# kuldeepbrd1/graspLDM

Measured on AMD Instinct MI355X. Metric: grasps/sec whole-node (1024-pt cloud, 100 DDIM steps), higher is better.
Workload: dtype f32 (GEMMs as split-f16 x3 partial products on the f16 matrix pipe, f32 accumulation; GroupNorm / LayerNorm / attention / scheduler in f32); 1 GPU; LDM mode, 256 synthetic 1024-pt clouds per GPU x 20 grasps, 100 DDIM steps: BASELINE.json configs[2] per GPU (configs[3] = this per-GPU workload on 8 GPUs); experiment=fpc, clouds_per_gpu=256, grasps_per_cloud=20, points=1024, ddim_steps=100, encoder=PVCNNEncoder (shipped fpc config), parallelism=cloud-sharded x1, weights=synthetic recipe seed 0, streams=3

## Files before the change

### graspldm_amd/csrc/quad_narrow.h

```cpp
#ifndef GLDM_QUAD_NARROW_H_
#define GLDM_QUAD_NARROW_H_

#ifdef GLDM_DEBUG_KNOBS
__device__ long long g_q_stamp[4][16];
#define GLDM_QSTAMP(c, i) do { if (blockIdx.x == 0 && (c).lane == 0) g_q_stamp[(c).wave & 3][i] = (long long)__builtin_readcyclecounter(); } while (0)
#else
#define GLDM_QSTAMP(c, i) do {} while (0)
#endif

template <int CTRL>
__device__ __forceinline__ float dpp_zero(float x) {
  return __int_as_float(__builtin_amdgcn_update_dpp(0, __float_as_int(x), CTRL, 0xf, 0xf, true));
}
template <int CTRL>
__device__ __forceinline__ u32x4 dpp_zero4(const u32x4 &v) {
  u32x4 o;
#pragma unroll
  for (int i = 0; i < 4; ++i) o[i] = (unsigned)__builtin_amdgcn_update_dpp(0, (int)v[i], CTRL, 0xf, 0xf, true);
  return o;
}
__device__ __forceinline__ float pos_sum(float v) {
  v += dpp_mov<0x124>(v);
  return v + dpp_mov<0x128>(v);
}
__device__ __forceinline__ float pos_max(float v) { return dpp_max<0x128>(dpp_max<0x124>(v)); }
#define GLDM_DPP8_STAGE1(op, i, j) "v_" op "_f32_dpp %" #i ", %" #j ", %" #j " row_ror:4 row_mask:0xf bank_mask:0xf\n\t"
#define GLDM_DPP8_STAGE2(op, i) "v_" op "_f32_dpp %" #i ", %" #i ", %" #i " row_ror:8 row_mask:0xf bank_mask:0xf\n\t"
#define GLDM_DPP8(op)                                                                                                  \
  "s_nop 1\n\t"                                                                                                         \
  GLDM_DPP8_STAGE1(op, 0, 8) GLDM_DPP8_STAGE1(op, 1, 9) GLDM_DPP8_STAGE1(op, 2, 10) GLDM_DPP8_STAGE1(op, 3, 11)          \
  GLDM_DPP8_STAGE1(op, 4, 12) GLDM_DPP8_STAGE1(op, 5, 13) GLDM_DPP8_STAGE1(op, 6, 14) GLDM_DPP8_STAGE1(op, 7, 15)        \
  GLDM_DPP8_STAGE2(op, 0) GLDM_DPP8_STAGE2(op, 1) GLDM_DPP8_STAGE2(op, 2) GLDM_DPP8_STAGE2(op, 3)                        \
  GLDM_DPP8_STAGE2(op, 4) GLDM_DPP8_STAGE2(op, 5) GLDM_DPP8_STAGE2(op, 6) GLDM_DPP8_STAGE2(op, 7)
#define GLDM_DPP8_OPERANDS                                                                                             \
  : "=&v"(r[0]), "=&v"(r[1]), "=&v"(r[2]), "=&v"(r[3]), "=&v"(r[4]), "=&v"(r[5]), "=&v"(r[6]), "=&v"(r[7])            \
  : "v"(x[0]), "v"(x[1]), "v"(x[2]), "v"(x[3]), "v"(x[4]), "v"(x[5]), "v"(x[6]), "v"(x[7])
#define GLDM_DPP8_STAGE1I(op, i) "v_" op "_f32_dpp %" #i ", %" #i ", %" #i " row_ror:4 row_mask:0xf bank_mask:0xf\n\t"
__device__ __forceinline__ void pos_max8(float (&x)[8]) {
  asm("s_nop 1\n\t"
      GLDM_DPP8_STAGE1I("max", 0) GLDM_DPP8_STAGE1I("max", 1) GLDM_DPP8_STAGE1I("max", 2) GLDM_DPP8_STAGE1I("max", 3)
      GLDM_DPP8_STAGE1I("max", 4) GLDM_DPP8_STAGE1I("max", 5) GLDM_DPP8_STAGE1I("max", 6) GLDM_DPP8_STAGE1I("max", 7)
      GLDM_DPP8_STAGE2("max", 0) GLDM_DPP8_STAGE2("max", 1) GLDM_DPP8_STAGE2("max", 2) GLDM_DPP8_STAGE2("max", 3)
      GLDM_DPP8_STAGE2("max", 4) GLDM_DPP8_STAGE2("max", 5) GLDM_DPP8_STAGE2("max", 6) GLDM_DPP8_STAGE2("max", 7)
      : "+v"(x[0]), "+v"(x[1]), "+v"(x[2]), "+v"(x[3]), "+v"(x[4]), "+v"(x[5]), "+v"(x[6]), "+v"(x[7]));
}
__device__ __forceinline__ void pos_sum8(const float (&x)[8], float (&r)[8]) {
  asm(GLDM_DPP8("add") GLDM_DPP8_OPERANDS);
}
__device__ __forceinline__ float kq_sum(float v) { return half_sum(row_pair_sum(v)); }
__device__ __forceinline__ float kq_max(float v) { return half_max(row_pair_max(v)); }

__device__ __forceinline__ void qsplit8(const f32x4 &a, const f32x4 &b, u32x4 (&pl)[kSplit]) {
  unsigned h, l;
  split_f16x2(a[0], a[1], h, l); pl[0][0] = h; pl[1][0] = l;
  split_f16x2(a[2], a[3], h, l); pl[0][1] = h; pl[1][1] = l;
  split_f16x2(b[0], b[1], h, l); pl[0][2] = h; pl[1][2] = l;
  split_f16x2(b[2], b[3], h, l); pl[0][3] = h; pl[1][3] = l;
}

enum { QM_OUT0 = 0, QM_SS2, QM_C1_2, QM_C2_2, QM_SS3, QM_C1_3, QM_C2_3, QM_QKV1, QM_OUT1, QM_DOWN1,
       QM_SS4, QM_C1_4, QM_C2_4, QM_SS5, QM_C1_5, QM_C2_5, QM_QKV2, QM_OUT2, QM_DOWN2, QM_COUNT };
struct QOff { int mat, a, b; };
constexpr QOff qconv_frag(int mat, int MT, int KB, int i, int mt0 = 0) {
  const int st = i / MT, mi = i % MT, kb = st / 3, t = st % 3;
  const int f = (mt0 + mi) * 3 * KB + t * KB + kb;
  return QOff{mat, 2048 * f, 2048 * f + 1024};
}
constexpr QOff qrb_frag(int mss, int MT, int KB, int i) {
  if (i < MT) return QOff{mss, 1024 * i, 1024 * (MT + i)};
  i -= MT;
  if (i < 3 * KB * MT) return qconv_frag(mss + 1, MT, KB, i);
  return qconv_frag(mss + 2, MT, KB, i - 3 * KB * MT);
}
constexpr int qrb_len(int MT, int KB) { return MT + 6 * KB * MT; }
constexpr QOff qatt_frag(int mqkv, int MT, int KB, int i) {
  const int per = 6 * KB + MT, h = i / per, r = i % per;
  if (r < 6 * KB) {
    const int mt6 = r / KB, kb = r % KB, part = mt6 / 2, half = mt6 % 2;
    const int f = (2 * h + half + 8 * part) * KB + kb;
    return QOff{mqkv, 2048 * f, 2048 * f + 1024};
  }
  const int f = (r - 6 * KB) * 4 + h;
  return QOff{mqkv + 1, 2048 * f, 2048 * f + 1024};
}
constexpr int qatt_len(int MT, int KB) { return 4 * (6 * KB + MT); }
constexpr int qlevel_len(int MT, int KB) { return 2 * qrb_len(MT, KB) + qatt_len(MT, KB) + 2 * MT * 3 * KB; }
constexpr QOff qlevel_frag(int m0, int MT, int KB, int DP, int i) {
  if (i < qrb_len(MT, KB)) return qrb_frag(m0, MT, KB, i);
  i -= qrb_len(MT, KB);
  if (i < qrb_len(MT, KB)) return qrb_frag(m0 + 3, MT, KB, i);
  i -= qrb_len(MT, KB);
  if (i < qatt_len(MT, KB)) return qatt_frag(m0 + 6, MT, KB, i);
  i -= qatt_len(MT, KB);
  const int pass = i / (DP * 3 * KB);
  return qconv_frag(m0 + 8, DP, KB, i % (DP * 3 * KB), DP * pass);
}
constexpr int kQN0 = 0;
constexpr int kQN1 = 4;
constexpr int kQN2 = kQN1 + qlevel_len(2, 1);
constexpr int kQNEnd = kQN2 + qlevel_len(4, 2);
constexpr QOff qstream_off(int n) {
  if (n < kQN1) return QOff{QM_OUT0, 2048 * n, 2048 * n + 1024};
  if (n < kQN2) return qlevel_frag(QM_SS2, 2, 1, 4, n - kQN1);
  return qlevel_frag(QM_SS4, 4, 2, 4, n - kQN2);
}

constexpr int kQG = 4;
constexpr int kQS = 32;
constexpr int kQGroups = kQNEnd / kQG;
static_assert(kQNEnd % kQG == 0 && kQS % kQG == 0, "whole groups");
constexpr int kQR = 6;
constexpr int kQSpinMax = 1 << 20;
__host__ __device__ constexpr int qslot_floats(int s) { return (s < 16 ? PG<4>::kH : PG<4>::kX + 4 * PG<4>::kBlockFloats) + (s & 15) * 512; }
static_assert(PG<4>::kH + 16 * 512 <= PG<4>::kX && PG<4>::kX + 4 * PG<4>::kBlockFloats + 16 * 512 <= 512 * 64, "slot regions");
typedef __attribute__((address_space(3))) int lds_i;
struct QStream4 {
  static constexpr int kEnd = kQNEnd, kGroups = kQGroups;
  static constexpr QOff off(int n) { return qstream_off(n); }
  __host__ __device__ static constexpr int slot_floats(int s) { return qslot_floats(s); }
};

struct QRing {
  u32x4 s[kQR][2];
  float *lds;
  lds_i *sync;
  int lane, quad;
  int flag;
  int spins = 0;
};
__device__ __forceinline__ int lds_poll(const lds_i *p) {
  int v;
  asm volatile("ds_read_b32 %0, %1\n\ts_waitcnt lgkmcnt(0)" : "=v"(v) : "v"(p) : "memory");
  return __builtin_amdgcn_readfirstlane(v);
}
template <int N, class ST = QStream4>
__device__ __forceinline__ void qring_load(QRing &ring) {
  if constexpr (N < ST::kEnd) {
    if constexpr (N % kQG == 0) {
      constexpr int g = N / kQG;
#if defined(GLDM_DEBUG_KNOBS) && defined(GLDM_QEXP_DUP)
      if (false) {
#else
      if (__builtin_expect(ring.flag != g + 1, 0)) {
#endif
        for (int spin = 0; spin < kQSpinMax && lds_poll(ring.sync + (g & 7)) != g + 1; ++spin) {
          __builtin_amdgcn_s_sleep(1);
#ifdef GLDM_DEBUG_KNOBS
          ++ring.spins;
#endif
        }
      }
      if constexpr (g + 1 < ST::kGroups) ring.flag = *(volatile lds_i *)(ring.sync + ((g + 1) & 7));
    }
#if defined(GLDM_DEBUG_KNOBS) && defined(GLDM_QEXP_NOLOAD)
    if (N >= kQR) return;
#endif
    const lds_u4 *slot = (const lds_u4 *)(ring.lds + ST::slot_floats(N % kQS)) + ring.lane;
    ring.s[N % kQR][0] = slot[0];
    ring.s[N % kQR][1] = slot[64];
  }
}
template <int N, class ST = QStream4>
__device__ __forceinline__ f32x4 qring_mfma(QRing &ring, const u32x4 (&b)[kSplit], f32x4 acc) {
#if defined(GLDM_DEBUG_KNOBS) && defined(GLDM_QEXP_NOMFMA)
  acc[0] += __uint_as_float(ring.s[N % kQR][0][0] ^ b[0][0]);
#else
  acc = mfma_split(ring.s[N % kQR], b, acc);
#endif
  if constexpr (N % kQG == kQG - 1) ring.sync[16 + 64 * ring.quad + ring.lane] = N / kQG + 1;
  if constexpr (N >= 1) qring_load<N - 1 + kQR, ST>(ring);
  return acc;
}

typedef __attribute__((address_space(3))) void lds_void;
typedef __attribute__((address_space(1))) const void glob_void;
__device__ __forceinline__ void quad_build_table(const gldm_r1d_desc &d, int *qtab, int tid, int nthreads) {
  const int mbf[QM_COUNT] = {d.lv[0].out_wq,
                             d.rb[2].ss_w, d.rb[2].c1_wq, d.rb[2].c2_wq, d.rb[3].ss_w, d.rb[3].c1_wq, d.rb[3].c2_wq,
                             d.lv[1].qkvn_wq, d.lv[1].out_wq, d.lv[1].down_wq,
                             d.rb[4].ss_w, d.rb[4].c1_wq, d.rb[4].c2_wq, d.rb[5].ss_w, d.rb[5].c1_wq, d.rb[5].c2_wq,
                             d.lv[2].qkvn_wq, d.lv[2].out_wq, d.lv[2].down_wq};
  for (int n = tid; n < kQNEnd; n += nthreads) {
    const QOff o = qstream_off(n);
    int base = 0;
#pragma unroll
    for (int m = 0; m < QM_COUNT; ++m) base = o.mat == m ? mbf[m] * 4 : base;
    qtab[2 * n] = base + o.a;
    qtab[2 * n + 1] = base + o.b;
  }
}
template <class ST = QStream4>
__device__ __forceinline__ void quad_loader(const Ctx &c) {
  using GG = Geo<64>;
  lds_i *sync = (lds_i *)(c.lds + GG::kMiscQ);
  const lds_i *qtab = (const lds_i *)(c.lds + GG::kMiscQTab);
  const char *wb = reinterpret_cast<const char *>(c.w) + c.lane * 16;
  for (int g = c.wave - 4; g < ST::kGroups; g += 4) {
    if (g >= 8) {
      for (int spin = 0; spin < kQSpinMax; ++spin) {
        const int d0 = lds_poll(sync + 16), d1 = lds_poll(sync + 80), d2 = lds_poll(sync + 144), d3 = lds_poll(sync + 208);
        if (min(min(d0, d1), min(d2, d3)) >= g - 7) break;
        __builtin_amdgcn_s_sleep(2);
      }
    }
    const int s0 = (g & 7) * kQG;
#pragma unroll
    for (int f = 0; f < kQG; ++f) {
      const int n = g * kQG + f;
      const int oa = __builtin_amdgcn_readfirstlane(qtab[2 * n]), ob = __builtin_amdgcn_readfirstlane(qtab[2 * n + 1]);
      const int sl = s0 + f;
      float *slot = c.lds + ST::slot_floats(sl);
      __builtin_amdgcn_global_load_lds((glob_void *)(wb + oa), (lds_void *)slot, 16, 0, 0);
      __builtin_amdgcn_global_load_lds((glob_void *)(wb + ob), (lds_void *)(slot + 256), 16, 0, 0);
    }
    asm volatile("s_waitcnt vmcnt(0)" ::: "memory");
    if (c.lane == 0) sync[g & 7] = g + 1;
  }
}

template <int N0, int MT, int KB, int SH = 4, class ST = QStream4>
__device__ __forceinline__ void qconv3(QRing &ring, const u32x4 (&xp)[KB][kSplit], f32x4 (&acc)[MT]) {
  using std::integral_constant;
  auto body = [&](auto st_c) {
    constexpr int st = decltype(st_c)::value, kb = st / 3, t = st % 3;
    u32x4 bs[kSplit];
#pragma unroll
    for (int pl = 0; pl < kSplit; ++pl)
      bs[pl] = t == 1 ? xp[kb][pl] : (t == 0 ? dpp_zero4<0x110 + SH>(xp[kb][pl]) : dpp_zero4<0x100 + SH>(xp[kb][pl]));
    auto per_m = [&](auto mi_c) {
      constexpr int mi = decltype(mi_c)::value;
      acc[mi] = qring_mfma<N0 + st * MT + mi, ST>(ring, bs, acc[mi]);
    };
    per_m(integral_constant<int, 0>{});
    if constexpr (MT > 1) per_m(integral_constant<int, 1>{});
    if constexpr (MT > 2) { per_m(integral_constant<int, 2>{}); per_m(integral_constant<int, 3>{}); }
    __builtin_amdgcn_sched_barrier(0);
  };
  body(integral_constant<int, 0>{}); body(integral_constant<int, 1>{}); body(integral_constant<int, 2>{});
  if constexpr (KB > 1) { body(integral_constant<int, 3>{}); body(integral_constant<int, 4>{}); body(integral_constant<int, 5>{}); }
}

template <int MT, int CPG>
__device__ __forceinline__ void qgn_stats(const f32x4 (&acc)[MT], float (&mean)[MT], float (&var)[MT]) {
  static_assert(CPG == 8 || CPG == 16, "groups of half an m-tile or a whole one");
  constexpr float inv_n = 1.0f / (float)(CPG * 4);
#pragma unroll
  for (int mi = 0; mi < MT; ++mi) {
    float s = (acc[mi][0] + acc[mi][1]) + (acc[mi][2] + acc[mi][3]);
    s = row_pair_sum(pos_sum(s));
    if (CPG == 16) s = half_sum(s);
    const float m = s * inv_n;
    float v = 0.f;
#pragma unroll
    for (int r = 0; r < 4; ++r) {
      const float d = acc[mi][r] - m;
      v = fmaf(d, d, v);
    }
    v = row_pair_sum(pos_sum(v));
    if (CPG == 16) v = half_sum(v);
    mean[mi] = m;
    var[mi] = v * inv_n;
  }
}

struct QRb { int c1_b, n1_w, n1_b, c2_b, n2_w, n2_b, ss_b; };

template <int N0, int MT, int KB>
__device__ __forceinline__ void quad_resblock(const Ctx &c, QRing &ring, const QRb &rb, f32x4 (&xr)[MT],
                                              u32x4 (&xp)[KB][kSplit], int smp) {
  using GG = Geo<64>;
  using std::integral_constant;
  constexpr int C = 16 * MT, CPG = C / 4;
  const int kq = c.lane >> 4;
  const float *w = c.w;
  const lds_f *Gs = (const lds_f *)(c.lds + GG::kMiscG) + smp * 16;
  float gb[4];
#pragma unroll
  for (int j = 0; j < 4; ++j) gb[j] = Gs[4 * j + kq];
  f32x4 sc[MT], sh[MT], g1[MT], be1[MT], b1[MT];
#pragma unroll
  for (int mi = 0; mi < MT; ++mi) {
    const int row0 = 16 * mi + 4 * kq;
    sc[mi] = *reinterpret_cast<const f32x4 *>(w + rb.ss_b + row0);
    sh[mi] = *reinterpret_cast<const f32x4 *>(w + rb.ss_b + C + row0);
    b1[mi] = *reinterpret_cast<const f32x4 *>(w + rb.c1_b + row0);
    g1[mi] = *reinterpret_cast<const f32x4 *>(w + rb.n1_w + row0);
    be1[mi] = *reinterpret_cast<const f32x4 *>(w + rb.n1_b + row0);
  }
  {
    auto ss_m = [&](auto mi_c) {
      constexpr int mi = decltype(mi_c)::value;
      const u32x4 a_sc = ring.s[(N0 + mi) % kQR][0], a_sh = ring.s[(N0 + mi) % kQR][1];
#pragma unroll
      for (int j = 0; j < 4; ++j) {
        sc[mi] = __builtin_amdgcn_mfma_f32_16x16x4f32(__uint_as_float(a_sc[j]), gb[j], sc[mi], 0, 0, 0);
        sh[mi] = __builtin_amdgcn_mfma_f32_16x16x4f32(__uint_as_float(a_sh[j]), gb[j], sh[mi], 0, 0, 0);
      }
      if constexpr (N0 + mi >= 1) qring_load<N0 + mi - 1 + kQR>(ring);
    };
    ss_m(integral_constant<int, 0>{}); ss_m(integral_constant<int, 1>{});
    if constexpr (MT > 2) { ss_m(integral_constant<int, 2>{}); ss_m(integral_constant<int, 3>{}); }
  }
// ... 218 lines not shown
  const int i = lane & 15, kq = lane >> 4;
  f32x4 f = *reinterpret_cast<const f32x4 *>(w + off + ((kq * 16 + (i >> 2)) * 4));
  if (i & 3) f = f32x4{0.f, 0.f, 0.f, 0.f};
  return f;
}
__device__ __forceinline__ float q4_conv(const f32x4 &wt, float bias, float x) {
  f32x4 acc = f32x4{bias, 0.f, 0.f, 0.f};
  acc = __builtin_amdgcn_mfma_f32_16x16x4f32(wt[0], dpp_zero<0x114>(x), acc, 0, 0, 0);
  acc = __builtin_amdgcn_mfma_f32_16x16x4f32(wt[1], x, acc, 0, 0, 0);
  acc = __builtin_amdgcn_mfma_f32_16x16x4f32(wt[2], dpp_zero<0x104>(x), acc, 0, 0, 0);
  return acc[0];
}
__device__ __forceinline__ float q4_gn(float y, float gamma, float beta) {
  const float m = pos_sum(y) * 0.25f;
  const float d = y - m;
  const float rs = __builtin_amdgcn_rsqf(pos_sum(d * d) * 0.25f + 1e-5f);
  return d * rs * gamma + beta;
}
struct QRb4W { f32x4 w1, w2, wss; float b1, g1, be1, b2, g2, be2, ssb0, ssb1; };
__device__ __forceinline__ QRb4W quad_resblock4_load(const Ctx &c, const QRb4 &rb) {
  const int i = c.lane & 15, kq = c.lane >> 4;
  const float *w = c.w;
  QRb4W p;
  p.w1 = q4_weights(w, rb.c1_w, c.lane);
  p.w2 = q4_weights(w, rb.c2_w, c.lane);
  const int srow = (i & 3) == 0 ? (i >> 2) : 4 + (i >> 2);
  p.wss = *reinterpret_cast<const f32x4 *>(w + rb.ss_w + ((kq * 16 + srow) * 4));
  if ((i & 3) > 1) p.wss = f32x4{0.f, 0.f, 0.f, 0.f};
  p.b1 = w[rb.c1_b + kq]; p.g1 = w[rb.n1_w + kq]; p.be1 = w[rb.n1_b + kq];
  p.b2 = w[rb.c2_b + kq]; p.g2 = w[rb.n2_w + kq]; p.be2 = w[rb.n2_b + kq];
  p.ssb0 = w[rb.ss_b + kq]; p.ssb1 = w[rb.ss_b + 4 + kq];
  return p;
}
__device__ __forceinline__ float quad_resblock4(const Ctx &c, const QRb4W &p, float x, int smp) {
  using GG = Geo<64>;
  const int kq = c.lane >> 4;
  f32x4 ss = f32x4{p.ssb0, p.ssb1, 0.f, 0.f};
  const lds_f *Gs = (const lds_f *)(c.lds + GG::kMiscG) + smp * 16;
#pragma unroll
  for (int j = 0; j < 4; ++j) ss = __builtin_amdgcn_mfma_f32_16x16x4f32(p.wss[j], Gs[4 * j + kq], ss, 0, 0, 0);
  float y = q4_conv(p.w1, p.b1, x);
  y = silu(q4_gn(y, p.g1, p.be1) * ss[0] + ss[1]);
  float z = q4_conv(p.w2, p.b2, y);
  z = silu(q4_gn(z, p.g2, p.be2));
  return x + z;
}

struct QLv4 { int qkvn_w, out_b, ln2_g; };

__device__ __forceinline__ float quad_attention4(const Ctx &c, QRing &ring, const QLv4 &lv, float x) {
  using std::integral_constant;
  const int kq = c.lane >> 4;
  const float *w = c.w;
  float fq[kHeads][6];
#pragma unroll
  for (int h = 0; h < kHeads; ++h)
#pragma unroll
    for (int t = 0; t < 6; ++t)
      fq[h][t] = w[lv.qkvn_w + ((2 * h + (t & 1) + 8 * (t >> 1)) * 64 + c.lane) * 4] * (t < 4 ? 1.44269504088896340736f : 1.0f);
  const float outb = w[lv.out_b + kq], g2 = w[lv.ln2_g + kq];
  const float mean = kq_sum(x) * 0.25f;
  const float d = x - mean;
  const float xn = d * __builtin_amdgcn_rsqf(kq_sum(d * d) * 0.25f + 1e-5f);
  f32x4 oacc = f32x4{outb, 0.f, 0.f, 0.f};
  auto head = [&](auto h_c) {
    constexpr int h = decltype(h_c)::value;
    f32x4 qkv[6];
#pragma unroll
    for (int t = 0; t < 6; ++t) qkv[t] = __builtin_amdgcn_mfma_f32_16x16x4f32(fq[h][t], xn, f32x4{0.f, 0.f, 0.f, 0.f}, 0, 0, 0);
    f32x4 o[2];
    const f32x4 qa[2] = {qkv[0], qkv[1]}, ka[2] = {qkv[2], qkv[3]}, va[2] = {qkv[4], qkv[5]};
    quad_attention_head<true>(qa, ka, va, o);
    u32x4 op[kSplit];
    qsplit8(o[0], o[1], op);
    oacc = qring_mfma<kQN0 + h>(ring, op, oacc);
  };
  head(integral_constant<int, 0>{}); head(integral_constant<int, 1>{}); head(integral_constant<int, 2>{}); head(integral_constant<int, 3>{});
  const float y = oacc[0];
  const float m2 = kq_sum(y) * 0.25f;
  const float d2 = y - m2;
  return x + d2 * __builtin_amdgcn_rsqf(kq_sum(d2 * d2) * 0.25f + 1e-5f) * g2;
}

typedef __attribute__((address_space(4))) const gldm_r1d_desc kernarg_desc;
#define GLDM_QDESC() asm volatile("" : "+s"(dk))
__device__ __forceinline__ void quad_narrow_levels(const Ctx &c, kernarg_desc *dk) {
  using GG = Geo<64>;
  using std::integral_constant;
  const int q = c.wave & 3, col = c.lane & 15, kq = c.lane >> 4;
  const int p = col >> 2, sl = col & 3;
  const int smp = 4 * q + sl;
  const int pmcol = 16 * p + smp;
  const float *w = c.w;
  QRing ring;
  ring.lds = c.lds;
  ring.sync = (lds_i *)(c.lds + GG::kMiscQ);
  ring.lane = c.lane;
  ring.quad = q;
  ring.flag = 0;
  GLDM_QSTAMP(c, 0);
  qring_load<0>(ring); qring_load<1>(ring); qring_load<2>(ring); qring_load<3>(ring); qring_load<4>(ring); qring_load<5>(ring);
  static_assert(kQR == 6, "priming loads");
#define GLDM_QRB4(i) QRb4{dk->rb[i].c1_w, dk->rb[i].c1_b, dk->rb[i].n1_w, dk->rb[i].n1_b, dk->rb[i].c2_w, dk->rb[i].c2_b, dk->rb[i].n2_w, dk->rb[i].n2_b, dk->rb[i].ss_w, dk->rb[i].ss_b}
#define GLDM_QRB(i) QRb{dk->rb[i].c1_b, dk->rb[i].n1_w, dk->rb[i].n1_b, dk->rb[i].c2_b, dk->rb[i].n2_w, dk->rb[i].n2_b, dk->rb[i].ss_b}
#define GLDM_QLV(i) QLv{dk->lv[i].qkvn_s, dk->lv[i].out_b, dk->lv[i].ln2_g}
  GLDM_QDESC();
  const QRb4W p0 = quad_resblock4_load(c, GLDM_QRB4(0)), p1 = quad_resblock4_load(c, GLDM_QRB4(1));
  float x = ((const lds_f *)(c.lds + GG::kBufX))[pswz(kq, pmcol)];
  x = quad_resblock4(c, p0, x, smp);
  GLDM_QSTAMP(c, 1);
  x = quad_resblock4(c, p1, x, smp);
  GLDM_QSTAMP(c, 2);
  GLDM_QDESC();
  x = quad_attention4(c, ring, QLv4{dk->lv[0].qkvn_w, dk->lv[0].out_b, dk->lv[0].ln2_g}, x);
  GLDM_QSTAMP(c, 3);
  f32x4 x32[2];
  u32x4 xp32[1][kSplit];
  {
    GLDM_QDESC();
    const WStream wd(w + dk->lv[0].down_w, c.lane);
    const float xl = dpp_zero<0x114>(x), xrr = dpp_zero<0x104>(x);
#pragma unroll
    for (int mi = 0; mi < 2; ++mi) {
      const f32x4 a = wd[(size_t)mi * 64];
      f32x4 acc = *reinterpret_cast<const f32x4 *>(w + dk->lv[0].down_b + 16 * mi + 4 * kq);
      acc = __builtin_amdgcn_mfma_f32_16x16x4f32(a[0], xl, acc, 0, 0, 0);
      acc = __builtin_amdgcn_mfma_f32_16x16x4f32(a[1], x, acc, 0, 0, 0);
      acc = __builtin_amdgcn_mfma_f32_16x16x4f32(a[2], xrr, acc, 0, 0, 0);
      x32[mi] = acc;
    }
    qsplit8(x32[0], x32[1], xp32[0]);
  }
  GLDM_QSTAMP(c, 4);
  constexpr int kRb1 = qrb_len(2, 1), kAtt1 = qatt_len(2, 1);
  GLDM_QDESC();
  quad_resblock<kQN1, 2, 1>(c, ring, GLDM_QRB(2), x32, xp32, smp);
  GLDM_QSTAMP(c, 5);
  GLDM_QDESC();
  quad_resblock<kQN1 + kRb1, 2, 1>(c, ring, GLDM_QRB(3), x32, xp32, smp);
  GLDM_QSTAMP(c, 6);
  GLDM_QDESC();
  quad_attention<kQN1 + 2 * kRb1, 2, 1>(c, ring, GLDM_QLV(1), x32, xp32);
  GLDM_QSTAMP(c, 7);
  f32x4 x64[4];
  u32x4 xp64[2][kSplit];
  {
    GLDM_QDESC();
    const int down_b1 = dk->lv[1].down_b;
#pragma unroll
    for (int mi = 0; mi < 4; ++mi) x64[mi] = *reinterpret_cast<const f32x4 *>(w + down_b1 + 16 * mi + 4 * kq);
    qconv3<kQN1 + 2 * kRb1 + kAtt1, 4, 1>(ring, xp32, x64);
    qsplit8(x64[0], x64[1], xp64[0]);
    qsplit8(x64[2], x64[3], xp64[1]);
  }
  GLDM_QSTAMP(c, 8);
  constexpr int kRb2 = qrb_len(4, 2), kAtt2 = qatt_len(4, 2);
  GLDM_QDESC();
  quad_resblock<kQN2, 4, 2>(c, ring, GLDM_QRB(4), x64, xp64, smp);
  GLDM_QSTAMP(c, 9);
  GLDM_QDESC();
  quad_resblock<kQN2 + kRb2, 4, 2>(c, ring, GLDM_QRB(5), x64, xp64, smp);
  GLDM_QSTAMP(c, 10);
  GLDM_QDESC();
  quad_attention<kQN2 + 2 * kRb2, 4, 2>(c, ring, GLDM_QLV(2), x64, xp64);
  GLDM_QSTAMP(c, 11);
  {
    lds_f *X3 = (lds_f *)(c.lds + GG::kBufX);
    GLDM_QDESC();
    const int down_b2 = dk->lv[2].down_b;
    auto pass = [&](auto h_c) {
      constexpr int half = decltype(h_c)::value;
      f32x4 acc[4];
#pragma unroll
      for (int mi = 0; mi < 4; ++mi) acc[mi] = *reinterpret_cast<const f32x4 *>(w + down_b2 + 16 * (4 * half + mi) + 4 * kq);
      qconv3<kQN2 + 2 * kRb2 + kAtt2 + 24 * half, 4, 2>(ring, xp64, acc);
#pragma unroll
      for (int mi = 0; mi < 4; ++mi) {
        const int row0 = 16 * (4 * half + mi) + 4 * kq;
#pragma unroll
        for (int r = 0; r < 4; ++r) X3[pswz(row0 + r, pmcol)] = acc[mi][r];
        store_planes4<4>(c.lds + PG<4>::kX, row0, pmcol, acc[mi][0], acc[mi][1], acc[mi][2], acc[mi][3]);
      }
    };
    pass(integral_constant<int, 0>{}); pass(integral_constant<int, 1>{});
  }
  GLDM_QSTAMP(c, 12);
#ifdef GLDM_DEBUG_KNOBS
  if (blockIdx.x == 0 && c.lane == 0) g_q_stamp[c.wave & 3][13] = ring.spins;
#endif
  static_assert(kQN2 + 2 * kRb2 + kAtt2 + 48 == kQNEnd, "stream length");
#undef GLDM_QDESC
#undef GLDM_QRB4
#undef GLDM_QRB
#undef GLDM_QLV
}

#endif
```

### graspldm_amd/csrc/r1d_debug.h

```cpp

#ifndef GLDM_R1D_DEBUG_DEVICE_PART
#define GLDM_R1D_DEBUG_DEVICE_PART

#if defined(GLDM_DEBUG_KNOBS) && defined(GLDM_WAVE_STAMPS)
__device__ long long g_wv_stamp[8][32][8];
__device__ int g_wv_cnt[8];
#define GLDM_WV_STAMP(c, k, v) \
  do { if (blockIdx.x == 0 && (c).lane == 0) g_wv_stamp[(c).wave][g_wv_cnt[(c).wave] & 31][k] = (v); } while (0)
#define GLDM_WV_NEXT(c) do { if (blockIdx.x == 0 && (c).lane == 0) g_wv_cnt[(c).wave]++; } while (0)
#else
#define GLDM_WV_STAMP(c, k, v) do {} while (0)
#define GLDM_WV_NEXT(c) do {} while (0)
#endif

#elif !defined(GLDM_DEBUG_KNOBS)

inline int dbg_slots(int slots) { return slots; }
inline size_t dbg_lds_bytes(size_t bytes) { return bytes; }
inline bool dbg_noquad() { return false; }
inline void dbg_arm(RunArgs &) {}
inline void dbg_report(const RunArgs &, bool, bool) {}

#else

inline int dbg_slots(int slots) {
  const char *e = getenv("GLDM_R1D_SLOTS");
  return e && atoi(e) > 0 ? atoi(e) : slots;
}
inline size_t dbg_lds_bytes(size_t bytes) {
  return getenv("GLDM_R1D_ONE_WG") && bytes < 100 * 1024 ? 100 * 1024 : bytes;
}
inline bool dbg_noquad() { return getenv("GLDM_R1D_NOQUAD") != nullptr; }

inline void dbg_arm(RunArgs &a) {
  const char *e = getenv("GLDM_R1D_SKIP");
  a.skip = e ? atoi(e) : 0;
  const char *g = getenv("GLDM_R1D_STAGGER_US");
  a.stagger_ticks = g ? atoi(g) * 100 : 0;
  static long long *dstamps = nullptr;
  const bool stamp = getenv("GLDM_R1D_STAMP") != nullptr;
  if (stamp && !dstamps) (void)hipMalloc(&dstamps, (kMaxOps + 2) * sizeof(long long));
  a.stamps = stamp ? dstamps : nullptr;
}

inline void dbg_report(const RunArgs &a, bool pm, bool pm16) {
  if (!a.stamps) return;
  static long long host[kMaxOps + 2];
  static int own_tape[kMaxOps * kOpInts];
  static const char *names[] = {"", "CONV", "RES4", "LN", "ATT", "QKVLN", "OUTLN", "QKVAT", "QUAD"};
  (void)hipDeviceSynchronize();
  (void)hipMemcpy(host, a.stamps, sizeof(host), hipMemcpyDeviceToHost);
  const int *tape = pm ? a.pm_tape : own_tape;
  const int n_ops = pm ? a.pm_nops : build_tape<kEngineNC>(a.d, own_tape);
  const bool quad = n_ops > 0 && tape[0] == OP_QUAD;
  for (int op = 0; op < n_ops; ++op) {
    const int *o = tape + kOpInts * op;
    int C = 0, cout = 0, taps = 0;
    switch (o[0]) {
      case OP_CONV: C = o[5]; cout = o[6]; taps = o[7] & 255; break;
      case OP_RES4: C = cout = 4; taps = 3; break;
      case OP_LN: C = cout = o[4]; break;
      case OP_ATT: C = (o - kOpInts)[5]; cout = 64; break;
      case OP_QKVATT: C = o[4]; cout = 384; taps = 1; break;
      case OP_OUTLN: C = o[5]; cout = o[6]; taps = 1; break;
      case OP_QUAD: C = a.d.dims[0]; cout = 128; taps = 3; break;
    }
    printf("op %3d %-5s C=%3d cout=%3d k=%d : %7lld clk\n", op, names[o[0]], C, cout, taps, host[op + 1] - host[op]);
  }
  printf("step total (ops): %lld clk; step prologue (embedding sums, init conv): %lld clk\n", host[n_ops] - host[0],
         host[0] - host[kMaxOps + 1]);
  if (quad) {
    static long long qs[4][16];
    (void)hipMemcpyFromSymbol(qs, HIP_SYMBOL(g_q_stamp), sizeof(qs));
    static const char *qn4[] = {"pads", "rb4", "rb4", "att4", "down4", "rb32", "rb32", "att32", "down32", "rb64", "rb64", "att64", "down64"};
    static const char *qn16[] = {"pads", "rb16", "rb16", "att16", "down16", "rb32", "rb32", "att32", "down32", "rb64", "rb64", "att64", "down64"};
    const char **qn = pm16 ? qn16 : qn4;
    for (int q = 0; q < 4; ++q) {
      printf("quad %d:", q);
      for (int i = 1; i <= 12; ++i) printf(" %s %lld", qn[i], qs[q][i] - qs[q][i - 1]);
      printf(" | total %lld, polls that waited %lld\n", qs[q][12] - qs[q][0], qs[q][13]);
    }
  }
#ifdef GLDM_WAVE_STAMPS
  if (pm) {
    static long long wv[8][32][8];
    int cnt[8];
    (void)hipMemcpyFromSymbol(wv, HIP_SYMBOL(g_wv_stamp), sizeof(wv));
    (void)hipMemcpyFromSymbol(cnt, HIP_SYMBOL(g_wv_cnt), sizeof(cnt));
    for (int i = 0; i < 32; ++i) {
      const int e = (cnt[0] + i) & 31;
      printf("conv %3lld->%3lld:", wv[0][e][3] / 1000, wv[0][e][3] % 1000);
      for (int w = 0; w < 8; ++w)
        printf("  w%d in %+5lld loop %6lld epi %6lld (stats %5lld wait %5lld finish %5lld) |", w, wv[w][e][0] - wv[0][e][0],
               wv[w][e][1] - wv[w][e][0], wv[w][e][2] - wv[w][e][1], wv[w][e][4] - wv[w][e][1], wv[w][e][5] - wv[w][e][4],
               wv[w][e][2] - wv[w][e][5]);
      printf("\n");
    }
  }
#endif
}

#endif
```

### graspldm_amd/csrc/resnet1d.hip

```cpp
#include "mfma_core.h"

namespace {

constexpr int kMaxSegs = 64;

#include "r1d_tape.h"
#include "r1d_debug.h"
#include "r1d_wide.h"
#include "r1d_rows.h"
#include "quad_narrow.h"
#include "quad16_narrow.h"
#include "r1d_chain.h"
#include "diffusion_step.h"

constexpr int kParkBytes = 256 * 64 * 4;

struct RunArgs {
  gldm_r1d_desc d;
  const float *weights;
  const float *temb;
  const float *cemb;
  const float *semb;
  int samples_per_cond;
  const float *x_in;
  int n_samples;
  const int32_t *timesteps;
  const int32_t *sample_t;
  int n_steps;
  int sched_kind, clip_sample;
  const float *sched_coef;
  const float *step_noise;
  unsigned long long noise_seed;
  long long noise_base;
  int noise_on;
  float *out0;
  float *out1;
  float *out2;
  const float *eps;
  float mix_mu, mix_eps;
  int eps_times_std;
  float *ws;
  float *park;
  const float *ss_tab;
  int ss_stride;
  int skip;
  int slots, rounds, left_tiles, chain, seglen;
  int stagger_ticks, n_cus;
  long long *stamps;
  int pm_nops;
  int pm_tape[kPmMaxOps * kOpInts];
};

template <int NC, int L>
__device__ __forceinline__ void run_tape(const Ctx &c0, const gldm_r1d_desc &d, const int *tape, kernarg_int *ktape, int n_ops, int E, long long *stamps) {
  constexpr bool KARG = NC == 64;
  for (int op = 0; op < n_ops; ++op) {
    if (stamps && c0.tid == 0) stamps[op] = (long long)__builtin_readcyclecounter();
    Ctx c = c0;
    asm volatile("" : "+v"(c.tid), "+v"(c.lane));
    int o[kOpInts];
    read_op<KARG>(tape, ktape, op, o);
    if (o[0] == OP_CONV && o[5] * o[6] >= 128 * 128) __builtin_amdgcn_s_setprio(0);
    else __builtin_amdgcn_s_setprio(3);
    switch (o[0]) {
      case OP_CONV: {
        if constexpr (NC == 64) {
          if (o[7] & kFlagFused) {
            int q[kOpInts];
            read_op<KARG>(tape, ktape, op + 1, q);
            const GnEpilogue g1{1, o[8], o[9], o[10], o[11], E, o[6], o[6] / 4, c.lds + o[4], (o[7] >> kFlagTabShift) << 2};
            const GnEpilogue g2{2, q[8], q[9], -1, 0, E, q[6], q[6] / 4, c.lds + q[4], 0};
            resblock_pm<L == 16 ? 16 : 4>(c, o[1], o[2], q[1], q[2], c.lds + o[3], c.lds + o[4], o[6], g1, g2, stamps ? stamps + op + 1 : nullptr);
            ++op;
            break;
          }
        }
        const int mode = GLDM_SKIP(c, 1) ? 0 : (o[7] >> 9) & 3;
        const GnEpilogue g{mode, o[8], o[9], GLDM_SKIP(c, 16) ? -1 : o[10], o[11], E, o[6], o[6] / 4, c.lds + o[4],
                           (o[7] >> kFlagTabShift) << 2};
        conv_gemm<NC, L>(c, o[1], o[2], c.lds + o[3], o[5], o[7] & 255, c.lds + o[4], o[6], (o[7] & kFlagAlias) != 0, 0, g);
        break;
      }
      case OP_QUAD:
        if constexpr (NC == 64 && L == 4) {
          if (c.wave < 4)
            quad_narrow_levels(c, (kernarg_desc *)((__attribute__((address_space(4))) const char *)__builtin_amdgcn_kernarg_segment_ptr() +
                                                    offsetof(RunArgs, d)));
#if defined(GLDM_DEBUG_KNOBS) && defined(GLDM_QEXP_DUP)
          else if (GLDM_QEXP_DUP == 2)
            quad_narrow_levels(c, (kernarg_desc *)((__attribute__((address_space(4))) const char *)__builtin_amdgcn_kernarg_segment_ptr() +
                                                    offsetof(RunArgs, d)));
#else
          else quad_loader(c);
#endif
          __syncthreads();
        } else if constexpr (NC == 64 && L == 16) {
          kernarg_desc *dkp = (kernarg_desc *)((__attribute__((address_space(4))) const char *)__builtin_amdgcn_kernarg_segment_ptr() +
                                               offsetof(RunArgs, d));
          const float *sstab;
          if (c.ss_lane) {
            const unsigned long long pv = (unsigned long long)c.ss_lane;
            const unsigned lo = (unsigned)__builtin_amdgcn_readlane((int)(unsigned)pv, c.wave & 3);
            const unsigned hi = (unsigned)__builtin_amdgcn_readlane((int)(unsigned)(pv >> 32), c.wave & 3);
            sstab = (const float *)(((unsigned long long)hi << 32) | lo);
          } else {
            quad16_ss_rows(c, dkp);
            __syncthreads();
            sstab = c.lds + kQ16SsLds + (c.wave & 3) * kQ16SsRows;
          }
          if (c.wave < 4) quad16_narrow_levels<1>(c, dkp, sstab);
          else quad_loader<QStream16<1>>(c);
          __syncthreads();
          zero_plane_pads16(c.lds, c.tid);
        }
        break;
      case OP_RES4:
        if (!GLDM_SKIP(c, 8)) {
          if constexpr (NC == 64 && L == 4) resblock4_pm(c, o, E);
          else if constexpr (NC != 64) resblock4_valu<NC>(c, o, E);
        }
        if (o[11]) __syncthreads();
        break;
      case OP_QKVATT:
        if constexpr (NC == 64) {
          if (o[4] == 128) {
            int q[kOpInts];
            read_op<KARG>(tape, ktape, op + 1, q);
            if (q[0] == OP_OUTLN && q[6] == 128) {
              const Frag3 first = out_ln_request(c, q[1]);
              if constexpr (L == 4) qkv_att_pm<4>(c, o[1], o[2], c.lds + o[3], o[4]);
              else qkv_att16_pm<4>(c, o[1], o[2], c.lds + o[3], o[4]);
              ++op;
              if (stamps && c0.tid == 0) stamps[op] = (long long)__builtin_readcyclecounter();
              out_ln_pm128<L == 16 ? 16 : 4>(c, q[1], q[2], c.lds + q[3], q[5], c.lds + q[4], q[7], first);
              break;
            }
          }
        }
        if constexpr (NC == 64 && L == 4) {
          if (o[4] == 128) qkv_att_pm<4>(c, o[1], o[2], c.lds + o[3], o[4]);
          else if (o[4] == 64) qkv_att_pm<2>(c, o[1], o[2], c.lds + o[3], o[4]);
          else if (o[4] == 32) qkv_att_pm<1>(c, o[1], o[2], c.lds + o[3], o[4]);
          else qkv_att_pm<0>(c, o[1], o[2], c.lds + o[3], o[4]);
        } else if constexpr (NC == 64 && L == 16) {
          if (o[4] == 128) qkv_att16_pm<4>(c, o[1], o[2], c.lds + o[3], o[4]);
          else if (o[4] == 64) qkv_att16_pm<2>(c, o[1], o[2], c.lds + o[3], o[4]);
          else qkv_att16_pm<1>(c, o[1], o[2], c.lds + o[3], o[4]);
        }
        break;
      case OP_OUTLN:
        if constexpr (NC == 64) out_ln_pm<L == 16 ? 16 : 4>(c, o[1], o[2], c.lds + o[3], o[5], c.lds + o[4], o[6], o[7]);
        break;
      case OP_LN:
        layer_norm_pass<NC>(c, c.lds + o[1], o[2] >= 0 ? c.lds + o[2] : nullptr, o[3] >= 0 ? c.lds + o[3] : nullptr,
                            o[4], o[5]);
        break;
      default:
        if constexpr (NC != 64) attention_pair<NC, L>(c, c.lds + o[1], c.lds + o[2]);
        break;
    }
  }
}

template <int NC, int L>
__global__ __launch_bounds__(Geo<NC>::kThreads, 2) void r1d_kernel(const RunArgs a) {
  using GG = Geo<NC>;
  extern __shared__ float lds[];
  const gldm_r1d_desc &d = a.d;
  constexpr int S = NC / L;
  constexpr bool PM = NC == 64;
  static_assert(!PM || L == 4 || L == 16, "64-column engines: 4- and 16-position nets");
  auto samp_of = [](int n) { return PM ? (L == 4 ? (n & 15) : (n & 3)) : n / L; };
  auto pos_of = [](int n) { return PM ? (L == 4 ? (n >> 4) : (n >> 2)) : n % L; };
  auto col_of = [](int sm, int l) { return PM ? (L == 4 ? 16 * l + sm : 4 * l + sm) : sm * L + l; };
  Ctx c{a.weights, lds, (int)threadIdx.x, __builtin_amdgcn_readfirstlane((int)threadIdx.x >> 6), (int)threadIdx.x & 63,
        a.skip, GG::kNT};
// ... 582 lines not shown
```

Baseline: 315,400 grasps/s.

## Split last down conv between quad waves and loader-helper waves

The last 64-wide down convolution's second half (m-tiles 4..7) moves from the four compute waves to the four loader waves. The loader waves now prefetch those weights straight into registers and receive the split input planes through a new LDS exchange area guarded by a flag. The weight stream shrinks by those 24 fragments, so the compute waves only run the first half. This shortens the critical path at the cost of an extra LDS handoff and spin-wait, plus higher register pressure in the helper waves.

New measurement: 317,100 grasps/s, median of 6. Within noise of the previous version (+0.5%).

```diff
diff --git a/graspldm_amd/csrc/quad_narrow.h b/graspldm_amd/csrc/quad_narrow.h
--- a/graspldm_amd/csrc/quad_narrow.h
+++ b/graspldm_amd/csrc/quad_narrow.h
@@ -4,8 +4,11 @@
 #ifdef GLDM_DEBUG_KNOBS
 __device__ long long g_q_stamp[4][16];
 #define GLDM_QSTAMP(c, i) do { if (blockIdx.x == 0 && (c).lane == 0) g_q_stamp[(c).wave & 3][i] = (long long)__builtin_readcyclecounter(); } while (0)
+__device__ long long g_qh_stamp[4][8];
+#define GLDM_QHSTAMP(c, i) do { if (blockIdx.x == 0 && (c).lane == 0) g_qh_stamp[(c).wave & 3][i] = (long long)__builtin_readcyclecounter(); } while (0)
 #else
 #define GLDM_QSTAMP(c, i) do {} while (0)
+#define GLDM_QHSTAMP(c, i) do {} while (0)
 #endif
 
 template <int CTRL>
@@ -98,7 +101,8 @@
 constexpr int kQN0 = 0;
 constexpr int kQN1 = 4;
 constexpr int kQN2 = kQN1 + qlevel_len(2, 1);
-constexpr int kQNEnd = kQN2 + qlevel_len(4, 2);
+constexpr int kQHelp = 4 * 3 * 2;
+constexpr int kQNEnd = kQN2 + qlevel_len(4, 2) - kQHelp;
 constexpr QOff qstream_off(int n) {
   if (n < kQN1) return QOff{QM_OUT0, 2048 * n, 2048 * n + 1024};
   if (n < kQN2) return qlevel_frag(QM_SS2, 2, 1, 4, n - kQN1);
@@ -113,6 +117,9 @@
 constexpr int kQSpinMax = 1 << 20;
 __host__ __device__ constexpr int qslot_floats(int s) { return (s < 16 ? PG<4>::kH : PG<4>::kX + 4 * PG<4>::kBlockFloats) + (s & 15) * 512; }
 static_assert(PG<4>::kH + 16 * 512 <= PG<4>::kX && PG<4>::kX + 4 * PG<4>::kBlockFloats + 16 * 512 <= 512 * 64, "slot regions");
+constexpr int kQExch = 512 * 64, kQExchFloats = 1024;
+static_assert(PG<4>::kX + 4 * PG<4>::kBlockFloats + 16 * 512 <= kQExch && kQExch + 4 * kQExchFloats <= Geo<64>::kArena,
+              "exchange areas: behind the ring, inside the arena");
 typedef __attribute__((address_space(3))) int lds_i;
 struct QStream4 {
   static constexpr int kEnd = kQNEnd, kGroups = kQGroups;
@@ -190,12 +197,13 @@
   }
 }
 template <class ST = QStream4>
-__device__ __forceinline__ void quad_loader(const Ctx &c) {
+__device__ __forceinline__ int quad_loader(const Ctx &c, int g0, int g_end) {
   using GG = Geo<64>;
   lds_i *sync = (lds_i *)(c.lds + GG::kMiscQ);
   const lds_i *qtab = (const lds_i *)(c.lds + GG::kMiscQTab);
   const char *wb = reinterpret_cast<const char *>(c.w) + c.lane * 16;
-  for (int g = c.wave - 4; g < ST::kGroups; g += 4) {
+  int g = g0;
+  for (; g < g_end; g += 4) {
     if (g >= 8) {
       for (int spin = 0; spin < kQSpinMax; ++spin) {
         const int d0 = lds_poll(sync + 16), d1 = lds_poll(sync + 80), d2 = lds_poll(sync + 144), d3 = lds_poll(sync + 208);
@@ -216,8 +224,26 @@
     asm volatile("s_waitcnt vmcnt(0)" ::: "memory");
     if (c.lane == 0) sync[g & 7] = g + 1;
   }
-}
-
+  return g;
+}
+template <class ST = QStream4>
+__device__ __forceinline__ void quad_loader(const Ctx &c) { quad_loader<ST>(c, c.wave - 4, ST::kGroups); }
+
+__device__ __forceinline__ void qflag_store(lds_i *p, int v) {
+  asm volatile("ds_write_b32 %0, %1" : : "v"(p), "v"(v) : "memory");
+}
+typedef __attribute__((address_space(4))) const gldm_r1d_desc kernarg_desc;
+typedef __attribute__((address_space(4))) const unsigned long long kernarg_u64;
+__device__ __forceinline__ int qflag_wait(const lds_i *p, int want, kernarg_desc *dk, int ws_off) {
+  int spin = 0;
+  for (; spin < kQSpinMax && lds_poll(p) < want; ++spin) __builtin_amdgcn_s_sleep(1);
+  if (__builtin_expect(spin == kQSpinMax, 0)) {
+    float *ws = reinterpret_cast<float *>(*(kernarg_u64 *)((__attribute__((address_space(4))) const char *)dk + ws_off));
+    if (ws) __hip_atomic_store(&reinterpret_cast<ChainHdr *>(ws)->error, 1u, __ATOMIC_RELAXED, __HIP_MEMORY_SCOPE_AGENT);
+  }
+  return spin;
+}
+constexpr int kQSeqDown64 = 1;
 template <int N0, int MT, int KB, int SH = 4, class ST = QStream4>
 __device__ __forceinline__ void qconv3(QRing &ring, const u32x4 (&xp)[KB][kSplit], f32x4 (&acc)[MT]) {
   using std::integral_constant;
@@ -602,7 +628,51 @@
   return x + d2 * __builtin_amdgcn_rsqf(kq_sum(d2 * d2) * 0.25f + 1e-5f) * g2;
 }
 
-typedef __attribute__((address_space(4))) const gldm_r1d_desc kernarg_desc;
+constexpr int kQHR = 16;
+struct QHelpW {
+  u32x4 f[kQHR][2];
+  const u32x4 *wd;
+  __device__ __forceinline__ void request(int i) {
+    const QOff o = qconv_frag(0, 4, 2, i, 4);
+    f[i % kQHR][0] = wd[o.a / 16];
+    f[i % kQHR][1] = wd[o.b / 16];
+  }
+};
+template <int N0, int HALF>
+__device__ __forceinline__ void quad_down128(const Ctx &c, QRing *ring, QHelpW *hw, f32x4 (&acc)[4], const u32x4 (&xp)[2][kSplit],
+                                             int kq, int pmcol) {
+  static_assert(kQHelp == 24 && kQHR == 16, "the helper's register ring");
+  using GG = Geo<64>;
+  using std::integral_constant;
+  lds_f *X3 = (lds_f *)(c.lds + GG::kBufX);
+  if constexpr (HALF == 0) {
+    qconv3<N0, 4, 2>(*ring, xp, acc);
+  } else {
+#pragma unroll
+    for (int st = 0; st < 6; ++st) {
+      const int kb = st / 3, t = st % 3;
+      u32x4 bs[kSplit];
+#pragma unroll
+      for (int pl = 0; pl < kSplit; ++pl)
+        bs[pl] = t == 1 ? xp[kb][pl] : (t == 0 ? dpp_zero4<0x114>(xp[kb][pl]) : dpp_zero4<0x104>(xp[kb][pl]));
+#pragma unroll
+      for (int mi = 0; mi < 4; ++mi) {
+        const int i = st * 4 + mi;
+        acc[mi] = mfma_split(hw->f[i % kQHR], bs, acc[mi]);
+        if (i >= 1 && i - 1 + kQHR < kQHelp) hw->request(i - 1 + kQHR);
+      }
+      __builtin_amdgcn_sched_barrier(0);
+    }
+  }
+#pragma unroll
+  for (int mi = 0; mi < 4; ++mi) {
+    const int row0 = 16 * (4 * HALF + mi) + 4 * kq;
+#pragma unroll
+    for (int r = 0; r < 4; ++r) X3[pswz(row0 + r, pmcol)] = acc[mi][r];
+    store_planes4<4>(c.lds + PG<4>::kX, row0, pmcol, acc[mi][0], acc[mi][1], acc[mi][2], acc[mi][3]);
+  }
+}
+
 #define GLDM_QDESC() asm volatile("" : "+s"(dk))
 __device__ __forceinline__ void quad_narrow_levels(const Ctx &c, kernarg_desc *dk) {
   using GG = Geo<64>;
@@ -685,34 +755,66 @@
   quad_attention<kQN2 + 2 * kRb2, 4, 2>(c, ring, GLDM_QLV(2), x64, xp64);
   GLDM_QSTAMP(c, 11);
   {
-    lds_f *X3 = (lds_f *)(c.lds + GG::kBufX);
+    lds_u4 *ex = (lds_u4 *)(c.lds + kQExch + kQExchFloats * q) + c.lane;
+    ex[0] = xp64[0][0]; ex[64] = xp64[0][1]; ex[128] = xp64[1][0]; ex[192] = xp64[1][1];
+    qflag_store(ring.sync + 8 + q, kQSeqDown64);
     GLDM_QDESC();
     const int down_b2 = dk->lv[2].down_b;
-    auto pass = [&](auto h_c) {
-      constexpr int half = decltype(h_c)::value;
-      f32x4 acc[4];
-#pragma unroll
-      for (int mi = 0; mi < 4; ++mi) acc[mi] = *reinterpret_cast<const f32x4 *>(w + down_b2 + 16 * (4 * half + mi) + 4 * kq);
-      qconv3<kQN2 + 2 * kRb2 + kAtt2 + 24 * half, 4, 2>(ring, xp64, acc);
-#pragma unroll
-      for (int mi = 0; mi < 4; ++mi) {
-        const int row0 = 16 * (4 * half + mi) + 4 * kq;
-#pragma unroll
-        for (int r = 0; r < 4; ++r) X3[pswz(row0 + r, pmcol)] = acc[mi][r];
-        store_planes4<4>(c.lds + PG<4>::kX, row0, pmcol, acc[mi][0], acc[mi][1], acc[mi][2], acc[mi][3]);
-      }
-    };
-    pass(integral_constant<int, 0>{}); pass(integral_constant<int, 1>{});
+    f32x4 acc[4];
+#pragma unroll
+    for (int mi = 0; mi < 4; ++mi) acc[mi] = *reinterpret_cast<const f32x4 *>(w + down_b2 + 16 * mi + 4 * kq);
+    quad_down128<kQN2 + 2 * kRb2 + kAtt2, 0>(c, &ring, nullptr, acc, xp64, kq, pmcol);
   }
   GLDM_QSTAMP(c, 12);
 #ifdef GLDM_DEBUG_KNOBS
   if (blockIdx.x == 0 && c.lane == 0) g_q_stamp[c.wave & 3][13] = ring.spins;
 #endif
-  static_assert(kQN2 + 2 * kRb2 + kAtt2 + 48 == kQNEnd, "stream length");
+  static_assert(kQN2 + 2 * kRb2 + kAtt2 + 24 == kQNEnd, "stream length");
 #undef GLDM_QDESC
 #undef GLDM_QRB4
 #undef GLDM_QRB
 #undef GLDM_QLV
 }
 
+__device__ __forceinline__ void quad_helper(const Ctx &c, kernarg_desc *dk, int ws_off) {
+  using GG = Geo<64>;
+  const int q = c.wave & 3, col = c.lane & 15, kq = c.lane >> 4;
+  const int pmcol = 16 * (col >> 2) + 4 * q + (col & 3);
+  lds_i *sync = (lds_i *)(c.lds + GG::kMiscQ);
+  const int g = quad_loader(c, q, kQGroups - 4);
+  asm volatile("" : "+s"(dk));
+  QHelpW hw;
+  hw.wd = reinterpret_cast<const u32x4 *>(c.w + dk->lv[2].down_wq) + c.lane;
+#pragma unroll
+  for (int i = 0; i < kQHR; ++i) hw.request(i);
+  f32x4 acc[4];
+  {
+    const int down_b2 = dk->lv[2].down_b;
+#pragma unroll
+    for (int mi = 0; mi < 4; ++mi) acc[mi] = *reinterpret_cast<const f32x4 *>(c.w + down_b2 + 16 * (4 + mi) + 4 * kq);
+  }
+  quad_loader(c, g, kQGroups);
+  GLDM_QHSTAMP(c, 0);
+#pragma unroll
+  for (int i = 0; i < kQHR; ++i) asm volatile("" : "+v"(hw.f[i][0]), "+v"(hw.f[i][1]));
+#pragma unroll
+  for (int mi = 0; mi < 4; ++mi) asm volatile("" : "+v"(acc[mi]));
+  GLDM_QHSTAMP(c, 1);
+  const int spins = qflag_wait(sync + 8 + q, kQSeqDown64, dk, ws_off);
+  GLDM_QHSTAMP(c, 2);
+  u32x4 xp[2][kSplit];
+  {
+    const lds_u4 *ex = (const lds_u4 *)(c.lds + kQExch + kQExchFloats * q) + c.lane;
+    xp[0][0] = ex[0]; xp[0][1] = ex[64]; xp[1][0] = ex[128]; xp[1][1] = ex[192];
+  }
+  quad_down128<0, 1>(c, nullptr, &hw, acc, xp, kq, pmcol);
+  GLDM_QHSTAMP(c, 3);
+#ifdef GLDM_DEBUG_KNOBS
+  if (blockIdx.x == 0 && c.lane == 0) g_qh_stamp[q][4] = spins;
+#else
+  (void)spins;
 #endif
+}
+static_assert(kQGroups >= 8 && qconv_frag(0, 4, 2, 0, 4).a == 2048 * 24, "the helper's fragments: m-tiles 4 .. 7 of the last down conv");
+
+#endif
diff --git a/graspldm_amd/csrc/r1d_debug.h b/graspldm_amd/csrc/r1d_debug.h
--- a/graspldm_amd/csrc/r1d_debug.h
+++ b/graspldm_amd/csrc/r1d_debug.h
@@ -80,6 +80,14 @@
       for (int i = 1; i <= 12; ++i) printf(" %s %lld", qn[i], qs[q][i] - qs[q][i - 1]);
       printf(" | total %lld, polls that waited %lld\n", qs[q][12] - qs[q][0], qs[q][13]);
     }
+    if (!pm16) {
+      static long long qh[4][8];
+      (void)hipMemcpyFromSymbol(qh, HIP_SYMBOL(g_qh_stamp), sizeof(qh));
+      for (int q = 0; q < 4; ++q)
+        printf("helper %d down64, from att64's end: loader duty done %+lld, weights in registers %+lld, planes seen %+lld, rows written %+lld "
+               "(quad's down64 end %+lld) | polls that waited %lld\n", q, qh[q][0] - qs[q][11], qh[q][1] - qs[q][11],
+               qh[q][2] - qs[q][11], qh[q][3] - qs[q][11], qs[q][12] - qs[q][11], qh[q][4]);
+    }
   }
 #ifdef GLDM_WAVE_STAMPS
   if (pm) {
diff --git a/graspldm_amd/csrc/resnet1d.hip b/graspldm_amd/csrc/resnet1d.hip
--- a/graspldm_amd/csrc/resnet1d.hip
+++ b/graspldm_amd/csrc/resnet1d.hip
@@ -8,9 +8,9 @@
 #include "r1d_debug.h"
 #include "r1d_wide.h"
 #include "r1d_rows.h"
+#include "r1d_chain.h"
 #include "quad_narrow.h"
 #include "quad16_narrow.h"
-#include "r1d_chain.h"
 #include "diffusion_step.h"
 
 constexpr int kParkBytes = 256 * 64 * 4;
@@ -83,6 +83,7 @@
       }
       case OP_QUAD:
         if constexpr (NC == 64 && L == 4) {
+          constexpr int kWsOff = (int)offsetof(RunArgs, ws) - (int)offsetof(RunArgs, d);
           if (c.wave < 4)
             quad_narrow_levels(c, (kernarg_desc *)((__attribute__((address_space(4))) const char *)__builtin_amdgcn_kernarg_segment_ptr() +
                                                     offsetof(RunArgs, d)));
@@ -91,7 +92,9 @@
             quad_narrow_levels(c, (kernarg_desc *)((__attribute__((address_space(4))) const char *)__builtin_amdgcn_kernarg_segment_ptr() +
                                                     offsetof(RunArgs, d)));
 #else
-          else quad_loader(c);
+          else
+            quad_helper(c, (kernarg_desc *)((__attribute__((address_space(4))) const char *)__builtin_amdgcn_kernarg_segment_ptr() +
+                                             offsetof(RunArgs, d)), kWsOff);
 #endif
           __syncthreads();
         } else if constexpr (NC == 64 && L == 16) {
```
